# yumingj/Text2Human

Measured on NVIDIA H100. Metric: 512x256 images/sec VQ enc-quant-dec (vqvae_top), higher is better.
Workload: dtype f32 (fp16x3 split products, fp32 accumulate)

## Files before the change

### include/t2h.h

```cpp
#ifndef T2H_H_
#define T2H_H_

#include <stdint.h>

#ifdef __cplusplus
extern "C" {
#endif

#define T2H_VERSION 202

#define T2H_OK 0
#define T2H_EINVAL (-1)
#define T2H_ECUDA (-2)
#define T2H_EARCH (-3)

typedef void* t2h_stream_t;

int t2h_version(void);
const char* t2h_last_error(void);
int t2h_device_info(int* cc_major, int* cc_minor, int* num_sms);

#define T2H_MAX_TAPS 16

#define T2H_OUT_F32 0
// ... 9 lines not shown
#define T2H_ACT_LRELU 3

typedef struct t2h_tapgemm_params {
  const void* a;
  int32_t a_terms;
  int32_t a_term_imgs;
  int32_t a_imgs;
  int32_t a_bcast;
  int32_t n_img, H, W;
  int32_t tile_rows;
  int32_t a_H, a_W;
  int32_t C;
  int64_t a_sw, a_sh, a_sn;
  const void* b;
  int32_t b_terms;
  int32_t b_term_g;
  int32_t b_groups;
  int32_t b_groups2;
  int32_t b_batched;
  int32_t b_batched_h;
  int32_t n_out;
  int64_t b_sn, b_sg, b_sg2;
  int32_t ntaps;
  int32_t tap_dy[T2H_MAX_TAPS];
  int32_t tap_dx[T2H_MAX_TAPS];
  int32_t tap_img_off[T2H_MAX_TAPS];
  int32_t nterms;
  void* d;
  int32_t d_mode;
  int32_t d_terms;
  int64_t d_plane;
  int64_t d_sn, d_sh, d_sw, d_sc;
  const float* bias;
  int32_t bias_mode;
  int32_t act;
  float alpha;
  const float* residual;
  double* gn_stats;
  int32_t gn_cpg;
  int32_t a_mn;
  int32_t b_mn;
  int64_t bias_sn;
  int32_t k_split;
  int32_t use_tap_w;
  int32_t tap_w[T2H_MAX_TAPS];
  int32_t accumulate;
  int32_t k_partials;
  int64_t d_slab;
  double* nb_sums;
  const double* nb_stats;
  const float* nb_gamma;
  const float* nb_beta;
  float nb_eps;
  int32_t nb_act;
  int32_t nb_groups;
} t2h_tapgemm_params;

int t2h_tapgemm(const t2h_tapgemm_params* p, t2h_stream_t stream);
int t2h_debug_read(long long* out, int n);

int t2h_nchw_to_planes(const float* x, void* out, int n, int c, int h, int w,
                       int c_pad, int terms, t2h_stream_t stream);
int t2h_nhwc_to_nchw(const float* x, float* out, int n, int c, int h, int w,
                     t2h_stream_t stream);
int t2h_pack_u8(const float* x, uint8_t* out, int n, int c, int h, int w, float scale, float shift,
                t2h_stream_t stream);
int t2h_nchw_to_nhwc(const float* x, float* out, int n, int c, int h, int w,
                     t2h_stream_t stream);

#define T2H_CVT_PLAIN 0
#define T2H_CVT_UP2X 1
#define T2H_CVT_S2D 2
#define T2H_CVT_MAXPOOL2 3
#define T2H_CVT_BILINEAR2X 4
int t2h_f32_to_planes(const float* x, void* out, int n, int h, int w, int c,
                      int mode, int terms, t2h_stream_t stream);

int t2h_gn_stats(const float* x, double* stats, int n, int hw, int c, int groups,
                 t2h_stream_t stream);
int t2h_gn_apply(const float* x, const double* stats, const float* gamma,
                 const float* beta, void* out, int n, int hw, int c, int groups,
                 float eps, int swish, int terms, t2h_stream_t stream);

int t2h_add_inplace(float* x, const float* y, int64_t numel, t2h_stream_t stream);

int t2h_softmax_rows(const float* s, void* out, int64_t rows, int cols, float scale,
                     int terms, t2h_stream_t stream);

int t2h_attn_fwd(const void* qkv, int terms, int64_t plane, int64_t ld, int64_t rows, int q_col, int k_col,
                 int v_col, int batch, int tokens, int heads, int head_dim, float scale, void* out,
                 int64_t out_plane, int64_t ld_out, t2h_stream_t stream);

int t2h_vq_search(const float* z, const float* codebook, const int32_t* book_id,
                  int b, int hz, int wz, int cz, int ps, int n_books, int n_e,
                  int64_t cont_stride, int64_t* idx, int64_t* idx_cont,
                  int64_t* idx_list, float* zq_nhwc, float* zq_nchw, double* sqerr,
                  void* workspace, int64_t workspace_bytes, t2h_stream_t stream);
int64_t t2h_vq_workspace_bytes(int64_t rows, int n_books, int n_e);

int t2h_vq_gather(const float* codebook, const int64_t* idx, const int32_t* book_id,
                  int b, int hz, int wz, int cz, int ps, int n_books, int n_e,
                  float* zq_nhwc, float* zq_nchw, t2h_stream_t stream);

int t2h_onehot_to_planes(const float* ids, void* out, int b, int h, int w, int n_classes, int c_pad, int terms,
                         t2h_stream_t stream);

int t2h_texture_mask(const float* segm, const int32_t* attrs, const int32_t* cls_group, int n_cls, float* mask, int b,
                     int64_t per_img, t2h_stream_t stream);
int t2h_u8_to_planes(const uint8_t* x, void* out, float* nchw, int b, int h, int w, int c, int c_pad, float divisor,
                     float shift, int terms, t2h_stream_t stream);

int t2h_mask_to_ids(const float* mask, int32_t* ids, int b, int hs, int ws, int ht,
                    int wt, t2h_stream_t stream);

int t2h_argmax_heads(const float* logits, const int64_t* head, int64_t* out, int64_t rows, int n_heads, int ncls,
                     t2h_stream_t stream);

int t2h_embed_sum(const int64_t* idx, const int64_t* segm, const int64_t* tex,
                  const float* tok_emb, const float* pos_emb, const float* segm_emb,
                  const float* tex_emb, float* x, int b, int t, int c,
                  t2h_stream_t stream);
int t2h_layernorm(const float* x, const float* gamma, const float* beta, void* out,
                  int64_t rows, int c, float eps, int terms, t2h_stream_t stream);
int t2h_layernorm_scatter(const float* x, const float* gamma, const float* beta, void* out, int64_t rows, int c,
                          float eps, int terms, const int64_t* row_map, int64_t out_rows, t2h_stream_t stream);

int t2h_splitk_reduce_ln(const float* partials, int n_slabs, int64_t slab, const float* bias, const float* residual,
                         float* x_out, const float* gamma, const float* beta, float eps, void* ln_out, int terms,
                         const int64_t* row_map, int64_t ln_rows, int64_t rows, int c, t2h_stream_t stream);

int t2h_f32_to_planes_t(const float* x, void* out_t, void* out_n, int g, int r, int c, int terms, float scale,
                        t2h_stream_t stream);
int t2h_planes_transpose(const void* x, void* out, int g, int r, int c, int64_t ld, int64_t g_stride,
                         int64_t in_plane, int64_t out_ld, int64_t out_g_stride, int64_t out_plane, int terms,
                         t2h_stream_t stream);
int t2h_colsum(const float* x, float* out, int64_t rows, int c, t2h_stream_t stream);
int t2h_gelu_fwd(const float* a, void* out, int64_t n, int terms, t2h_stream_t stream);
int t2h_gelu_bwd(const float* a, const float* dg, float* da, void* da_planes ,
                 int64_t n, int terms, t2h_stream_t stream);
int t2h_layernorm_bwd(const float* dy, const float* x, const float* gamma, float* dx, float* dgamma,
                      float* dbeta, int64_t rows, int c, float eps, int accumulate, t2h_stream_t stream);
int t2h_layernorm_bwd_fused(const float* dy, const float* x, const float* gamma, float* dx, float* dgamma,
                            float* dbeta, int64_t rows, int c, float eps, int accumulate, void* dx_planes, int terms,
                            float* dx_colsum, t2h_stream_t stream);
int t2h_softmax_bwd(const void* p, const float* dp, float* ds, int64_t rows, int cols, float scale, int terms,
                    t2h_stream_t stream);
int t2h_softmax_bwd_planes(const void* p, const float* dp, void* ds_planes, int64_t rows, int cols, float scale,
                           int terms, float out_scale, t2h_stream_t stream);
int t2h_ce_heads(const float* logits, const int64_t* target, const int64_t* head, const float* w,
                 float* loss_rows, float* dlogits, int64_t rows, int nh, int ncls, t2h_stream_t stream);
int t2h_embed_bwd(const float* dx, const int64_t* idx, float* de, int64_t rows, int c, int t_mod,
                  t2h_stream_t stream);
int t2h_adam(float* p, const float* g, float* m, float* v, int64_t n, float lr, float beta1, float beta2,
             float eps, int step, float grad_scale, t2h_stream_t stream);

typedef struct t2h_conv_wgrad_params {
  const void* dy;
  int32_t dy_terms, dy_term_imgs, dy_imgs;
  int32_t n_img, H, W, cout;
  int64_t dy_sw, dy_sh, dy_sn;
  const void* x;
  int32_t x_terms, x_term_imgs, x_imgs;
  int32_t x_H, x_W, cin;
  int64_t x_sw, x_sh, x_sn;
  int32_t ntaps;
  int32_t tap_dy[T2H_MAX_TAPS], tap_dx[T2H_MAX_TAPS], tap_img_off[T2H_MAX_TAPS];
// ... 44 lines not shown
```

### text2human_b200/_lib.py

```python
import ctypes as C
import os

_HERE = os.path.dirname(os.path.abspath(__file__))
LIB_PATH = os.path.join(_HERE, "libt2h.so")

ABI_VERSION = 202
MAX_TAPS = 16
OUT_F32, OUT_PLANES = 0, 1
BIAS_NONE, BIAS_COL, BIAS_ROW = 0, 1, 2
ACT_NONE, ACT_GELU, ACT_RELU, ACT_LRELU = 0, 1, 2, 3
CVT_PLAIN, CVT_UP2X, CVT_S2D, CVT_MAXPOOL2, CVT_BILINEAR2X = 0, 1, 2, 3, 4


class TapGemmParams(C.Structure):
    _fields_ = [
        ("a", C.c_void_p), ("a_terms", C.c_int32), ("a_term_imgs", C.c_int32),
        ("a_imgs", C.c_int32), ("a_bcast", C.c_int32),
        ("n_img", C.c_int32), ("H", C.c_int32), ("W", C.c_int32), ("tile_rows", C.c_int32),
        ("a_H", C.c_int32), ("a_W", C.c_int32), ("C", C.c_int32),
        ("a_sw", C.c_int64), ("a_sh", C.c_int64), ("a_sn", C.c_int64),
        ("b", C.c_void_p), ("b_terms", C.c_int32), ("b_term_g", C.c_int32),
        ("b_groups", C.c_int32), ("b_groups2", C.c_int32), ("b_batched", C.c_int32),
        ("b_batched_h", C.c_int32), ("n_out", C.c_int32),
        ("b_sn", C.c_int64), ("b_sg", C.c_int64), ("b_sg2", C.c_int64),
        ("ntaps", C.c_int32),
        ("tap_dy", C.c_int32 * MAX_TAPS), ("tap_dx", C.c_int32 * MAX_TAPS),
        ("tap_img_off", C.c_int32 * MAX_TAPS),
        ("nterms", C.c_int32),
        ("d", C.c_void_p), ("d_mode", C.c_int32), ("d_terms", C.c_int32),
        ("d_plane", C.c_int64),
        ("d_sn", C.c_int64), ("d_sh", C.c_int64), ("d_sw", C.c_int64), ("d_sc", C.c_int64),
        ("bias", C.c_void_p), ("bias_mode", C.c_int32), ("act", C.c_int32),
        ("alpha", C.c_float),
        ("residual", C.c_void_p),
        ("gn_stats", C.c_void_p), ("gn_cpg", C.c_int32), ("a_mn", C.c_int32), ("b_mn", C.c_int32), ("bias_sn", C.c_int64), ("k_split", C.c_int32),
        ("use_tap_w", C.c_int32), ("tap_w", C.c_int32 * MAX_TAPS), ("accumulate", C.c_int32),
        ("k_partials", C.c_int32), ("d_slab", C.c_int64),
        ("nb_sums", C.c_void_p), ("nb_stats", C.c_void_p), ("nb_gamma", C.c_void_p), ("nb_beta", C.c_void_p),
        ("nb_eps", C.c_float), ("nb_act", C.c_int32), ("nb_groups", C.c_int32),
    ]


class ConvWgradParams(C.Structure):
    _fields_ = [
        ("dy", C.c_void_p), ("dy_terms", C.c_int32), ("dy_term_imgs", C.c_int32), ("dy_imgs", C.c_int32),
        ("n_img", C.c_int32), ("H", C.c_int32), ("W", C.c_int32), ("cout", C.c_int32),
        ("dy_sw", C.c_int64), ("dy_sh", C.c_int64), ("dy_sn", C.c_int64),
        ("x", C.c_void_p), ("x_terms", C.c_int32), ("x_term_imgs", C.c_int32), ("x_imgs", C.c_int32),
        ("x_H", C.c_int32), ("x_W", C.c_int32), ("cin", C.c_int32),
        ("x_sw", C.c_int64), ("x_sh", C.c_int64), ("x_sn", C.c_int64),
        ("ntaps", C.c_int32),
        ("tap_dy", C.c_int32 * MAX_TAPS), ("tap_dx", C.c_int32 * MAX_TAPS), ("tap_img_off", C.c_int32 * MAX_TAPS),
        ("dw", C.c_void_p), ("dw_tap_stride", C.c_int64), ("dw_ld", C.c_int64),
        ("alpha", C.c_float), ("nterms", C.c_int32), ("k_split", C.c_int32),
    ]


_I, _L, _P, _F = C.c_int, C.c_int64, C.c_void_p, C.c_float
SIGNATURES = {
    "t2h_version": (_I, []),
    "t2h_last_error": (C.c_char_p, []),
    "t2h_device_info": (_I, [C.POINTER(_I)] * 3),
    "t2h_tapgemm": (_I, [C.POINTER(TapGemmParams), _P]),
    "t2h_debug_read": (_I, [C.POINTER(C.c_longlong), _I]),
    "t2h_nchw_to_planes": (_I, [_P, _P, _I, _I, _I, _I, _I, _I, _P]),
    "t2h_nhwc_to_nchw": (_I, [_P, _P, _I, _I, _I, _I, _P]),
    "t2h_nchw_to_nhwc": (_I, [_P, _P, _I, _I, _I, _I, _P]),
    "t2h_f32_to_planes": (_I, [_P, _P, _I, _I, _I, _I, _I, _I, _P]),
    "t2h_gn_stats": (_I, [_P, _P, _I, _I, _I, _I, _P]),
    "t2h_gn_apply": (_I, [_P, _P, _P, _P, _P, _I, _I, _I, _I, _F, _I, _I, _P]),
    "t2h_add_inplace": (_I, [_P, _P, _L, _P]),
    "t2h_softmax_rows": (_I, [_P, _P, _L, _I, _F, _I, _P]),
    "t2h_attn_fwd": (_I, [_P, _I, _L, _L, _L, _I, _I, _I, _I, _I, _I, _I, _F, _P, _L, _L, _P]),
    "t2h_vq_search": (_I, [_P, _P, _P, _I, _I, _I, _I, _I, _I, _I, _L, _P, _P, _P, _P, _P, _P,
                           _P, _L, _P]),
    "t2h_vq_workspace_bytes": (_L, [_L, _I, _I]),
    "t2h_vq_gather": (_I, [_P, _P, _P, _I, _I, _I, _I, _I, _I, _I, _P, _P, _P]),
    "t2h_texture_mask": (_I, [_P, _P, _P, _I, _P, _I, _L, _P]),
    "t2h_u8_to_planes": (_I, [_P, _P, _P, _I, _I, _I, _I, _I, _F, _F, _I, _P]),
    "t2h_mask_to_ids": (_I, [_P, _P, _I, _I, _I, _I, _I, _P]),
    "t2h_onehot_to_planes": (_I, [_P, _P, _I, _I, _I, _I, _I, _I, _P]),
    "t2h_embed_sum": (_I, [_P, _P, _P, _P, _P, _P, _P, _P, _I, _I, _I, _P]),
    "t2h_layernorm": (_I, [_P, _P, _P, _P, _L, _I, _F, _I, _P]),
    "t2h_layernorm_scatter": (_I, [_P, _P, _P, _P, _L, _I, _F, _I, _P, _L, _P]),
    "t2h_splitk_reduce_ln": (_I, [_P, _I, _L, _P, _P, _P, _P, _P, _F, _P, _I, _P, _L, _L, _I, _P]),
    "t2h_pack_u8": (_I, [_P, _P, _I, _I, _I, _I, _F, _F, _P]),
    "t2h_argmax_heads": (_I, [_P, _P, _P, _L, _I, _I, _P]),
    "t2h_f32_to_planes_t": (_I, [_P, _P, _P, _I, _I, _I, _I, _F, _P]),
    "t2h_planes_transpose": (_I, [_P, _P, _I, _I, _I, _L, _L, _L, _L, _L, _L, _I, _P]),
    "t2h_colsum": (_I, [_P, _P, _L, _I, _P]),
    "t2h_gelu_fwd": (_I, [_P, _P, _L, _I, _P]),
    "t2h_gelu_bwd": (_I, [_P, _P, _P, _P, _L, _I, _P]),
    "t2h_layernorm_bwd_fused": (_I, [_P, _P, _P, _P, _P, _P, _L, _I, _F, _I, _P, _I, _P, _P]),
    "t2h_softmax_bwd_planes": (_I, [_P, _P, _P, _L, _I, _F, _I, _F, _P]),
    "t2h_layernorm_bwd": (_I, [_P, _P, _P, _P, _P, _P, _L, _I, _F, _I, _P]),
    "t2h_softmax_bwd": (_I, [_P, _P, _P, _L, _I, _F, _I, _P]),
    "t2h_ce_heads": (_I, [_P, _P, _P, _P, _P, _P, _L, _I, _I, _P]),
    "t2h_embed_bwd": (_I, [_P, _P, _P, _L, _I, _I, _P]),
    "t2h_adam": (_I, [_P, _P, _P, _P, _L, _F, _F, _F, _F, _I, _F, _P]),
    "t2h_conv_wgrad": (_I, [C.POINTER(ConvWgradParams), _P]),
    "t2h_norm_bwd": (_I, [_P, _P, _P, _P, _P, _P, _P, _P, _I, _P, _P, _P, _I, _I, _I, _I, _F, _I, _P, _I, _P]),
    "t2h_bn_update_running": (_I, [_P, _P, _P, _L, _F, _I, _P]),
    "t2h_lrelu_bwd": (_I, [_P, _P, _P, _P, _I, _L, _P]),
    "t2h_sumpool2": (_I, [_P, _P, _I, _I, _I, _I, _P]),
    "t2h_planes_s2d": (_I, [_P, _P, _I, _I, _I, _I, _I, _P]),
    "t2h_vq_bwd": (_I, [_P, _P, _P, _P, _P, _P, _P, _L, _I, _I, _I, _F, _F, _P]),
    "t2h_l1_loss": (_I, [_P, _P, _P, _P, _L, _F, _P]),
    "t2h_bce_logits": (_I, [_P, _P, _I, _I, _I, _I, _I, _F, _P, _P, _I, _P, _P]),
    "t2h_hinge_loss": (_I, [_P, _P, _P, _L, _F, _F, _P]),
    "t2h_diffaug_fwd": (_I, [_P, _P, _P, _P, _P, _I, _I, _I, _P]),
    "t2h_diffaug_bwd": (_I, [_P, _P, _P, _P, _P, _I, _I, _I, _P]),
    "t2h_adaptive_weight": (_I, [_P, _P, _L, _F, _F, _F, _P, _P]),
    "t2h_axpy_dev": (_I, [_P, _P, _P, _P, _L, _P]),
    "t2h_sample_step": (_I, [_P, _P, _P, _P, _P, _L, _I, _I, _F, _F, C.c_uint64, C.c_uint32, _L, _P]),
}

_lib = None


class T2HError(RuntimeError):
    pass


def load():
    global _lib
    if _lib is not None:
        return _lib
    if not os.path.exists(LIB_PATH):
        raise T2HError(
            f"{LIB_PATH} not found: build it with `python -c 'import __graft_entry__ as g; g.build()'` "
            "(or `make -C text2human_b200/csrc`). There is no CPU fallback.")
    lib = C.CDLL(LIB_PATH)
    for name, (res, args) in SIGNATURES.items():
        fn = getattr(lib, name)
        fn.restype = res
        fn.argtypes = args
    _lib = lib
    return lib


def check(rc):
    if rc != 0:
        raise T2HError(f"libt2h error {rc}: {load().t2h_last_error().decode()}")
```

### text2human_b200/ops.py

```python
import ctypes as C

import torch

from . import _lib
from ._lib import (ACT_GELU, ACT_LRELU, ACT_NONE, ACT_RELU, CVT_BILINEAR2X, CVT_MAXPOOL2, BIAS_COL, BIAS_NONE, BIAS_ROW, CVT_PLAIN, CVT_S2D, CVT_UP2X,
                   OUT_F32, OUT_PLANES, TapGemmParams)

_PRECISION = {"terms": 2, "mixed": False}


def set_precision(mode):
    _PRECISION["mixed"] = False
    if mode in ("fp32", "fp16x3", "exact"):
        _PRECISION["terms"] = 2
    elif mode in ("fp16", "fast", "tf32"):
        _PRECISION["terms"] = 1
    elif mode == "mixed":
        _PRECISION["terms"] = 2
        _PRECISION["mixed"] = True
    else:
        raise ValueError(f"unknown precision mode {mode!r}")


def layer_terms(mod):
# ... 353 lines not shown
    assert K == Kb and a.stride(3) == 1 and b.stride(3) == 1
    assert (Ga == G) or (a_bcast and Ga == 1)
    out = _alloc_out((G, M, N), planes_out, T, a.device)
    a_sn = a.stride(1)
    a_term_imgs = 1 if T == 1 else a.stride(0) // a_sn
    assert T == 1 or a.stride(0) % a_sn == 0
    _tapgemm(a=a, a_term_imgs=a_term_imgs, a_imgs=(T - 1) * a_term_imgs + Ga, a_bcast=1 if a_bcast else 0,
             n_img=G, H=1, W=M, a_H=1, a_W=M, Cc=K, a_sw=a.stride(2), a_sh=a_sn, a_sn=a_sn,
             b=b, b_term_g=1, b_groups=Tb, b_sg=b.stride(0), b_groups2=G, b_sg2=b.stride(1), b_batched=1,
             n_out=N, b_sn=b.stride(2),
             taps=_TAPS_1, d=out, d_mode=OUT_PLANES if planes_out else OUT_F32,
             d_strides=(M * N, 0, N, 1), d_plane=G * M * N,
             bias=bias_row if bias_col is None else bias_col,
             bias_mode=BIAS_ROW if bias_col is None else BIAS_COL,
             bias_sn=0 if bias_col is None else N, alpha=alpha, act=act)
    return out


def mha_scores(q, B, Tn, nh, alpha=1.0, k=None):
    if k is None:
        Cc = q.shape[2] // 2
        q, k = q[:, :, :Cc], q[:, :, Cc:]
    _need_cuda(q, k)
    T, M, Cc = q.shape
    hs = Cc // nh
    assert M == B * Tn and k.shape == q.shape and q.stride(2) == 1 and k.stride(2) == 1
    ldq, ldk = q.stride(1), k.stride(1)
    out = torch.empty((B, nh, Tn, Tn), dtype=torch.float32, device=q.device)
    plane = q.stride(0)
    assert plane % hs == 0 and (T == 1 or k.stride(0) == M * ldk)
    _tapgemm(a=q, a_term_imgs=plane // hs, a_imgs=(T - 1) * (plane // hs) + nh, a_bcast=0,
             n_img=nh, H=B, W=Tn, a_H=B, a_W=Tn, Cc=hs, a_sw=ldq, a_sh=Tn * ldq, a_sn=hs, tile_rows=1,
             b=k, b_term_g=B, b_groups=T * B, b_sg=Tn * ldk, b_batched_h=1,
             b_groups2=nh, b_sg2=hs, b_batched=1, n_out=Tn, b_sn=ldk,
             taps=_TAPS_1, d=out, d_mode=OUT_F32, d_strides=(Tn * Tn, nh * Tn * Tn, Tn, 1), alpha=alpha)
    return out


def mha_pv(p, vt, B, Tn, nh, out=None, planes_out=True, alpha=1.0, p_mn=False, v_tok=False):
    _need_cuda(p, vt)
    T = p.shape[0]
    assert p.is_contiguous()
    if v_tok:
        Cc = vt.shape[2]
        ldv = vt.stride(1)
        assert vt.shape[1] == B * Tn and vt.stride(2) == 1 and (T == 1 or vt.stride(0) == B * Tn * ldv)
        b_kw = dict(b_sg=Tn * ldv, b_sg2=Cc // nh, b_sn=ldv, b_mn=1)
    else:
        Cc = vt.shape[2]
        assert vt.is_contiguous()
        b_kw = dict(b_sg=Cc * Tn, b_sg2=(Cc // nh) * Tn, b_sn=Tn, b_mn=0)
    hs = Cc // nh
    if out is None:
        out = _alloc_out((B * Tn, Cc), planes_out, T, p.device)
    ld = out.stride(-2)
    _tapgemm(a=p, a_term_imgs=B * nh, a_imgs=T * B * nh, a_bcast=0,
             n_img=nh, H=B, W=Tn, a_H=B, a_W=Tn, Cc=Tn, a_sw=Tn, a_sh=nh * Tn * Tn, a_sn=Tn * Tn,
             tile_rows=1,
             b=vt, b_term_g=B, b_groups=T * B, b_batched_h=1,
             b_groups2=nh, b_batched=1, n_out=hs,
             taps=_TAPS_1, d=out, d_mode=OUT_PLANES if planes_out else OUT_F32, d_strides=(hs, Tn * ld, ld, 1),
             d_plane=out.stride(0) if planes_out else 0, alpha=alpha, a_mn=1 if p_mn else 0, **b_kw)
    return out


def split_planes(x, terms):
    x = x.detach().float()
    hi = x.half()
    if terms == 1:
        return hi.unsqueeze(0).contiguous()
    lo = (x - hi.float()).half()
    return torch.stack((hi, lo)).contiguous()


def pack_conv_weight(w, terms, c_pad=None):
    Cout, Cin, kh, kw = w.shape
    wt = w.detach().float().permute(2, 3, 0, 1).reshape(kh * kw, Cout, Cin)
    cp = c_pad if c_pad is not None else (Cin + 7) // 8 * 8
    if cp != Cin:
        wt = torch.nn.functional.pad(wt, (0, cp - Cin))
    return split_planes(wt, terms)


def conv_weight_for_dgrad(w):
    return w.detach().flip(2, 3).transpose(0, 1).contiguous()


def pack_linear_weight(w, terms):
    w2 = w.detach().float().reshape(w.shape[0], -1)
    return split_planes(w2.unsqueeze(0), terms)


def nchw_to_planes(x, c_pad=None, terms=None):
    _need_cuda(x)
    x = _f32c(x)
    N, Cc, H, W = x.shape
    terms = terms or get_terms()
    cp = c_pad if c_pad is not None else (Cc + 7) // 8 * 8
    out = torch.empty((terms, N, H, W, cp), dtype=torch.float16, device=x.device)
    _count(1)
    _lib.check(_lib.load().t2h_nchw_to_planes(_ptr(x), _ptr(out), N, Cc, H, W, cp, terms, _stream()))
    return out


def nhwc_to_nchw(x):
    _need_cuda(x)
    N, H, W, Cc = x.shape
    out = torch.empty((N, Cc, H, W), dtype=torch.float32, device=x.device)
    _count(1)
    _lib.check(_lib.load().t2h_nhwc_to_nchw(_ptr(x), _ptr(out), N, Cc, H, W, _stream()))
    return out


def nchw_to_nhwc(x):
    _need_cuda(x)
    x = _f32c(x)
    N, Cc, H, W = x.shape
    out = torch.empty((N, H, W, Cc), dtype=torch.float32, device=x.device)
    _count(1)
    _lib.check(_lib.load().t2h_nchw_to_nhwc(_ptr(x), _ptr(out), N, Cc, H, W, _stream()))
    return out


def f32_to_planes(x, mode=CVT_PLAIN, terms=None):
    _need_cuda(x)
    N, H, W, Cc = x.shape
    terms = terms or get_terms()
    if mode in (CVT_UP2X, CVT_BILINEAR2X):
        shape = (terms, N, 2 * H, 2 * W, Cc)
    elif mode == CVT_MAXPOOL2:
        shape = (terms, N, H // 2, W // 2, Cc)
    elif mode == CVT_S2D:
        shape = (terms, 4, N, H // 2, W // 2, Cc)
    else:
        shape = (terms, N, H, W, Cc)
    out = torch.empty(shape, dtype=torch.float16, device=x.device)
    _count(1)
    _lib.check(_lib.load().t2h_f32_to_planes(_ptr(x), _ptr(out), N, H, W, Cc, mode, terms, _stream()))
    return out


def group_norm(x, gamma, beta, *, swish, groups=32, eps=1e-6, terms=None, stats=None):
    _need_cuda(x)
    N, H, W, Cc = x.shape
    terms = terms or get_terms()
    lib = _lib.load()
    _count(1)
    if stats is None:
        stats = torch.zeros((N, groups, 2), dtype=torch.float64, device=x.device)
        _count(1)
        _lib.check(lib.t2h_gn_stats(_ptr(x), _ptr(stats), N, H * W, Cc, groups, _stream()))
    out = torch.empty((terms, N, H, W, Cc), dtype=torch.float16, device=x.device)
    _lib.check(lib.t2h_gn_apply(_ptr(x), _ptr(stats), _ptr(gamma), _ptr(beta), _ptr(out), N, H * W, Cc,
                                groups, eps, 1 if swish else 0, terms, _stream()))
    return out


def add_inplace(x, y):
    _need_cuda(x, y)
    assert x.shape == y.shape and x.is_contiguous() and y.is_contiguous()
    _count(1)
    _lib.check(_lib.load().t2h_add_inplace(_ptr(x), _ptr(y), x.numel(), _stream()))
    return x


def softmax_rows(s, scale=1.0, terms=None):
    _need_cuda(s)
    terms = terms or get_terms()
    cols = s.shape[-1]
    rows = s.numel() // cols
    out = torch.empty((terms,) + tuple(s.shape), dtype=torch.float16, device=s.device)
    _count(1)
    _lib.check(_lib.load().t2h_softmax_rows(_ptr(s), _ptr(out), rows, cols, scale, terms, _stream()))
    return out


FUSED_ATTN = {"on": _os_env.environ.get("T2H_FUSED_ATTN", "1") != "0"}


def set_fused_attn(on):
    old = FUSED_ATTN["on"]
    FUSED_ATTN["on"] = bool(on)
    return old


def can_fuse_attn(tokens, head_dim):
    return FUSED_ATTN["on"] and head_dim == 64 and tokens % 128 == 0 and 128 <= tokens <= 512


def attn_fused(qkv, B, Tn, nh, scale, out=None):
    _need_cuda(qkv)
    T, M, C3 = qkv.shape
    Cc = C3 // 3
    assert M == B * Tn and Cc == nh * 64 and qkv.stride(2) == 1 and qkv.dtype == torch.float16
    if out is None:
        out = torch.empty((T, M, Cc), dtype=torch.float16, device=qkv.device)
    assert out.shape == (T, M, Cc) and out.stride(2) == 1
    _count(1)
    _lib.check(_lib.load().t2h_attn_fwd(_ptr(qkv), T, qkv.stride(0), qkv.stride(1), M, 0, Cc, 2 * Cc, B, Tn, nh, 64,
                                        float(scale), _ptr(out), out.stride(0), out.stride(1), _stream()))
    return out


def layer_norm(x, gamma, beta, eps=1e-5, terms=None):
    _need_cuda(x)
    terms = terms or get_terms()
    rows, Cc = x.shape
    out = torch.empty((terms, rows, Cc), dtype=torch.float16, device=x.device)
    _count(1)
    _lib.check(_lib.load().t2h_layernorm(_ptr(x), _ptr(gamma), _ptr(beta), _ptr(out), rows, Cc, eps, terms,
                                         _stream()))
    return out


def layer_norm_scatter(x, gamma, beta, out, row_map, eps=1e-5):
    _need_cuda(x, out, row_map)
    rows, Cc = x.shape
    assert out.is_contiguous() and out.shape[2] == Cc and row_map.dtype == torch.int64 and row_map.numel() == rows
    _count(1)
    _lib.check(_lib.load().t2h_layernorm_scatter(_ptr(x), _ptr(gamma), _ptr(beta), _ptr(out), rows, Cc, eps,
                                                 out.shape[0], _ptr(row_map), out.shape[1], _stream()))
    return out


def embed_sum(idx, segm, tex, tok_emb, pos_emb, segm_emb, tex_emb):
    _need_cuda(idx, tok_emb)
    B, T = idx.shape
    Cc = tok_emb.shape[1]
    x = torch.empty((B * T, Cc), dtype=torch.float32, device=idx.device)
    _count(1)
    _lib.check(_lib.load().t2h_embed_sum(_ptr(idx.contiguous()), _ptr(segm.contiguous()),
                                         _ptr(tex.contiguous()), _ptr(tok_emb), _ptr(pos_emb),
                                         _ptr(segm_emb), _ptr(tex_emb), _ptr(x), B, T, Cc, _stream()))
    return x


def onehot_to_planes(segm, n_classes, terms=None):
# ... 499 lines not shown
```

### text2human_b200/vqgan_arch.py

```python
import numpy as np
import torch
import torch.nn as nn

from . import ops
from .ops import CVT_PLAIN, CVT_S2D, CVT_UP2X


def _cached(owner, key, params, build):
    cache = owner.__dict__.setdefault("_t2h_cache", {})
    sig = tuple((p.data_ptr(), p._version, str(p.device)) for p in params)
    hit = cache.get(key)
    if hit is not None and hit[0] == sig:
        return hit[1]
    with torch.no_grad():
        val = build()
    cache[key] = (sig, val)
    return val


def _conv_w(conv, c_pad=None):
    t = ops.layer_terms(conv)
    return _cached(conv, ("w3", t, c_pad), (conv.weight,),
                   lambda: ops.pack_conv_weight(conv.weight, t, c_pad))

# ... 92 lines not shown
        out_channels = in_channels if out_channels is None else out_channels
        self.out_channels = out_channels
        self.use_conv_shortcut = conv_shortcut

        self.norm1 = Normalize(in_channels)
        self.conv1 = torch.nn.Conv2d(in_channels, out_channels, kernel_size=3, stride=1, padding=1)
        if temb_channels > 0:
            self.temb_proj = torch.nn.Linear(temb_channels, out_channels)
        self.norm2 = Normalize(out_channels)
        self.dropout = torch.nn.Dropout(dropout)
        self.conv2 = torch.nn.Conv2d(out_channels, out_channels, kernel_size=3, stride=1, padding=1)
        if self.in_channels != self.out_channels:
            if self.use_conv_shortcut:
                self.conv_shortcut = torch.nn.Conv2d(in_channels, out_channels, kernel_size=3, stride=1,
                                                     padding=1)
            else:
                self.nin_shortcut = torch.nn.Conv2d(in_channels, out_channels, kernel_size=1, stride=1,
                                                    padding=0)

    def _fwd(self, act):
        assert self.dropout.p == 0.0 or not self.training, "dropout>0 in training is not implemented"
        x = act.x
        h = _Act(*_gn_conv3x3(act, self.norm1, self.conv1, want_stats=True))
        if self.in_channels != self.out_channels:
            xp = ops.f32_to_planes(x, CVT_PLAIN)
            if self.use_conv_shortcut:
                x = ops.conv3x3(xp, _conv_w(self.conv_shortcut), _f32(self.conv_shortcut.bias))
            else:
                x = conv1x1_nhwc(None, self.nin_shortcut, planes_in=xp)
        return _Act(*_gn_conv3x3(h, self.norm2, self.conv2, residual=x, want_stats=True))

    def forward_nhwc(self, x, temb=None):
        assert temb is None, "temb is always None on the Text2Human path (temb_ch=0)"
        return self._fwd(_Act(x)).x

    def forward(self, x, temb=None):
        return ops.nhwc_to_nchw(self.forward_nhwc(ops.nchw_to_nhwc(x), temb))


class AttnBlock(nn.Module):

    def __init__(self, in_channels):
        super().__init__()
        self.in_channels = in_channels
        self.norm = Normalize(in_channels)
        self.q = torch.nn.Conv2d(in_channels, in_channels, kernel_size=1, stride=1, padding=0)
        self.k = torch.nn.Conv2d(in_channels, in_channels, kernel_size=1, stride=1, padding=0)
        self.v = torch.nn.Conv2d(in_channels, in_channels, kernel_size=1, stride=1, padding=0)
        self.proj_out = torch.nn.Conv2d(in_channels, in_channels, kernel_size=1, stride=1, padding=0)

    def _qk_packed(self):
        t = ops.get_terms()
        w = _cached(self, ("wqk", t), (self.q.weight, self.k.weight),
                    lambda: ops.pack_linear_weight(torch.cat((self.q.weight, self.k.weight), 0), t))
        b = _cached(self, ("bqk",), (self.q.bias, self.k.bias),
                    lambda: torch.cat((self.q.bias, self.k.bias), 0).float().contiguous())
        return w, b

    def _fwd(self, act):
        x = act.x
        N, H, W, Cc = x.shape
        HW = H * W
        hn = _gn(act, self.norm, swish=False)
        T = hn.shape[0]
        wqk, bqk = self._qk_packed()
        qk = ops.linear(hn.reshape(T, N * HW, Cc), wqk, bqk, planes_out=True).view(T, N, HW, 2 * Cc)
        q, k = qk[..., :Cc], qk[..., Cc:]
        vt = ops.bmm_nt(_lin_w(self.v), hn.view(T, N, HW, Cc), planes_out=True,
                        bias_row=_f32(self.v.bias), a_bcast=True)
        s = ops.bmm_nt(q, k)
        p = ops.softmax_rows(s, scale=float(int(Cc) ** (-0.5)))
        o = ops.bmm_nt(p, vt, planes_out=True)
        return _Act(*ops.conv1x1(o.view(T, N, H, W, Cc), _lin_w(self.proj_out), _f32(self.proj_out.bias),
                                 residual=x, want_stats=True))

    def forward_nhwc(self, x):
        return self._fwd(_Act(x)).x

    def forward(self, x):
        return ops.nhwc_to_nchw(self.forward_nhwc(ops.nchw_to_nhwc(x)))


def _conv_in_nchw(conv, x):
    a = ops.nchw_to_planes(x)
    return _Act(*ops.conv3x3(a, _conv_w(conv, a.shape[-1]), _f32(conv.bias), want_stats=True))


def _conv_in_nhwc(conv, x):
    a = ops.f32_to_planes(x, CVT_PLAIN)
    return _Act(*ops.conv3x3(a, _conv_w(conv), _f32(conv.bias), want_stats=True))


def _conv_out(norm, conv, act, nchw):
    return _gn_conv3x3(act, norm, conv, nchw_out=nchw)


class Encoder(nn.Module):

    def __init__(self, ch, num_res_blocks, attn_resolutions, in_channels, resolution, z_channels,
                 ch_mult=(1, 2, 4, 8), dropout=0.0, resamp_with_conv=True, double_z=True):
        super().__init__()
        self.ch = ch
        self.temb_ch = 0
        self.num_resolutions = len(ch_mult)
        self.num_res_blocks = num_res_blocks
        self.resolution = resolution
        self.in_channels = in_channels

        self.conv_in = torch.nn.Conv2d(in_channels, self.ch, kernel_size=3, stride=1, padding=1)

        curr_res = resolution
        in_ch_mult = (1, ) + tuple(ch_mult)
        self.down = nn.ModuleList()
        for i_level in range(self.num_resolutions):
            block = nn.ModuleList()
            attn = nn.ModuleList()
            block_in = ch * in_ch_mult[i_level]
            block_out = ch * ch_mult[i_level]
            for _ in range(self.num_res_blocks):
                block.append(ResnetBlock(in_channels=block_in, out_channels=block_out,
                                         temb_channels=self.temb_ch, dropout=dropout))
                block_in = block_out
                if curr_res in attn_resolutions:
                    attn.append(AttnBlock(block_in))
            down = nn.Module()
            down.block = block
            down.attn = attn
            if i_level != self.num_resolutions - 1:
                down.downsample = Downsample(block_in, resamp_with_conv)
                curr_res = curr_res // 2
            self.down.append(down)

        self.mid = nn.Module()
        self.mid.block_1 = ResnetBlock(in_channels=block_in, out_channels=block_in,
                                       temb_channels=self.temb_ch, dropout=dropout)
        self.mid.attn_1 = AttnBlock(block_in)
        self.mid.block_2 = ResnetBlock(in_channels=block_in, out_channels=block_in,
                                       temb_channels=self.temb_ch, dropout=dropout)

        self.norm_out = Normalize(block_in)
        self.conv_out = torch.nn.Conv2d(block_in, 2 * z_channels if double_z else z_channels,
                                        kernel_size=3, stride=1, padding=1)

    def _body(self, h):
        for i_level in range(self.num_resolutions):
            lvl = self.down[i_level]
            for i_block in range(self.num_res_blocks):
                h = lvl.block[i_block]._fwd(h)
                if len(lvl.attn) > 0:
                    h = lvl.attn[i_block]._fwd(h)
            if i_level != self.num_resolutions - 1:
                h = lvl.downsample._fwd(h)
        h = self.mid.block_1._fwd(h)
        h = self.mid.attn_1._fwd(h)
        h = self.mid.block_2._fwd(h)
        return h

    @torch.no_grad()
    def forward_planes(self, a):
        h = _Act(*ops.conv3x3(a, _conv_w(self.conv_in, a.shape[-1]), _f32(self.conv_in.bias), want_stats=True))
        return _conv_out(self.norm_out, self.conv_out, self._body(h), nchw=False)

    @torch.no_grad()
    def forward_nhwc(self, x_nchw):
        h = self._body(_conv_in_nchw(self.conv_in, x_nchw))
        return _conv_out(self.norm_out, self.conv_out, h, nchw=False)

    def forward(self, x):
        from . import vqgan_autograd as VA
        if VA.recording(self, x):
            return VA.encoder_forward(self, x)
        with torch.no_grad():
            h = self._body(_conv_in_nchw(self.conv_in, x))
            return _conv_out(self.norm_out, self.conv_out, h, nchw=True)


# ... 334 lines not shown
```

Measured before the change: 201.5.

## Add fused GN-swish small-Cout conv and im2col path for first conv

For output convs with at most three channels, a new CUDA-core kernel fuses GroupNorm apply and swish with a direct fp32 3x3 convolution. This avoids materializing normalized fp16 planes and running a tensor-core GEMM that would waste most of its N dimension. For input convs with few channels, the NCHW input is turned into im2col fp16 planes so the conv runs as a single-tap GEMM with a dense K dimension instead of a padded 9-tap one. The small-Cout path computes in plain fp32 FMAs instead of split fp16 products, which shifts numerics slightly, and it adds an extra im2col buffer.

```diff
diff --git a/include/t2h.h b/include/t2h.h
--- a/include/t2h.h
+++ b/include/t2h.h
@@ -115,6 +115,13 @@
                  const float* beta, void* out, int n, int hw, int c, int groups,
                  float eps, int swish, int terms, t2h_stream_t stream);
 
+int t2h_gn_swish_conv3x3_small(const float* x, const double* stats, const float* gamma, const float* beta, float eps,
+                               const float* wpk, const float* bias, float* out, int n, int h, int w, int c, int cout,
+                               int groups, long long o_sn, long long o_sh, long long o_sw, long long o_sc,
+                               t2h_stream_t stream);
+int t2h_nchw_im2col_planes(const float* x, void* out, int n, int c, int h, int w, int k_pad, int terms,
+                           t2h_stream_t stream);
+
 int t2h_add_inplace(float* x, const float* y, int64_t numel, t2h_stream_t stream);
 
 int t2h_softmax_rows(const float* s, void* out, int64_t rows, int cols, float scale,
diff --git a/text2human_b200/_lib.py b/text2human_b200/_lib.py
--- a/text2human_b200/_lib.py
+++ b/text2human_b200/_lib.py
@@ -69,6 +69,8 @@
     "t2h_f32_to_planes": (_I, [_P, _P, _I, _I, _I, _I, _I, _I, _P]),
     "t2h_gn_stats": (_I, [_P, _P, _I, _I, _I, _I, _P]),
     "t2h_gn_apply": (_I, [_P, _P, _P, _P, _P, _I, _I, _I, _I, _F, _I, _I, _P]),
+    "t2h_gn_swish_conv3x3_small": (_I, [_P, _P, _P, _P, _F, _P, _P, _P, _I, _I, _I, _I, _I, _I, _L, _L, _L, _L, _P]),
+    "t2h_nchw_im2col_planes": (_I, [_P, _P, _I, _I, _I, _I, _I, _I, _P]),
     "t2h_add_inplace": (_I, [_P, _P, _L, _P]),
     "t2h_softmax_rows": (_I, [_P, _P, _L, _I, _F, _I, _P]),
     "t2h_attn_fwd": (_I, [_P, _I, _L, _L, _L, _I, _I, _I, _I, _I, _I, _I, _F, _P, _L, _L, _P]),
diff --git a/text2human_b200/csrc/conv_small.cu b/text2human_b200/csrc/conv_small.cu
--- /dev/null
+++ b/text2human_b200/csrc/conv_small.cu
@@ -0,0 +1,206 @@
+#include "t2h_internal.h"
+#include "t2h_ptx.cuh"
+
+namespace t2h {
+
+constexpr int kSW = 32, kSR = 8, kSWarps = 8, kSH = kSR * kSWarps, kSC = 8;
+constexpr int kSTileW = kSW + 2, kSTileH = kSH + 2, kSPix = kSTileW * kSTileH, kSPlane = kSPix;
+constexpr int kSThreads = kSWarps * 32;
+static_assert(kSPlane % 32 == 4 && kSC == 8, "activation plane stride: the two quads of a pixel 16 banks apart");
+
+template <int COUT>
+__global__ void __launch_bounds__(kSThreads, 3)
+gn_swish_conv3x3_small_kernel(const float* __restrict__ x, const double* __restrict__ stats,
+                              const float* __restrict__ gamma, const float* __restrict__ beta, float eps,
+                              const float* __restrict__ wpk, const float* __restrict__ bias, float* __restrict__ out,
+                              int H, int W, int C, int groups, long long o_sn, long long o_sh, long long o_sw,
+                              long long o_sc) {
+  extern __shared__ __align__(16) float sm[];
+  float* s_act = sm;
+  float* s_w = s_act + kSC * kSPlane;
+  float* s_scale = s_w + kSC * 36;
+  float* s_shift = s_scale + C;
+  const int n = blockIdx.z;
+  const int h0 = blockIdx.y * kSH, w0 = blockIdx.x * kSW;
+  const int tid = threadIdx.x, lane = tid & 31, warp = tid >> 5;
+
+  const int cpg = C / groups;
+  const double cnt = (double)H * W * cpg;
+  for (int c = tid; c < C; c += kSThreads) {
+    const int g = c / cpg;
+    const double s = stats[((long long)n * groups + g) * 2 + 0];
+    const double q = stats[((long long)n * groups + g) * 2 + 1];
+    const double mean = s / cnt;
+    double var = q / cnt - mean * mean;
+    if (var < 0) var = 0;
+    const float rstd = (float)(1.0 / sqrt(var + (double)eps));
+    const float ga = gamma[c] * rstd;
+    s_scale[c] = ga;
+    s_shift[c] = beta[c] - (float)mean * ga;
+  }
+
+  float acc[kSR][COUT];
+#pragma unroll
+  for (int o = 0; o < kSR; ++o)
+#pragma unroll
+    for (int co = 0; co < COUT; ++co) acc[o][co] = 0.f;
+
+  const float* xn = x + (long long)n * H * W * C;
+  for (int c0 = 0; c0 < C; c0 += kSC) {
+    __syncthreads();
+    for (int i = tid; i < kSC * 9; i += kSThreads)
+      reinterpret_cast<float4*>(s_w)[i] = __ldg(reinterpret_cast<const float4*>(wpk + (long long)c0 * 36) + i);
+#pragma unroll 4
+    for (int i = tid; i < kSPix * (kSC / 4); i += kSThreads) {
+      const int q = i & (kSC / 4 - 1), p = i / (kSC / 4);
+      const int r = p / kSTileW, col = p - r * kSTileW;
+      const int gh = h0 + r - 1, gw = w0 + col - 1;
+      float f[4] = {0.f, 0.f, 0.f, 0.f};
+      if (gh >= 0 && gh < H && gw >= 0 && gw < W) {
+        const float4 a = __ldg(reinterpret_cast<const float4*>(xn + ((long long)gh * W + gw) * C + c0) + q);
+        f[0] = a.x; f[1] = a.y; f[2] = a.z; f[3] = a.w;
+#pragma unroll
+        for (int e = 0; e < 4; ++e) {
+          const float y = f[e] * s_scale[c0 + 4 * q + e] + s_shift[c0 + 4 * q + e];
+          f[e] = y / (1.0f + __expf(-y));
+        }
+      }
+#pragma unroll
+      for (int e = 0; e < 4; ++e) s_act[(4 * q + e) * kSPlane + p] = f[e];
+    }
+    __syncthreads();
+#pragma unroll 1
+    for (int e = 0; e < kSC; ++e) {
+      float4 wv[9];
+#pragma unroll
+      for (int k = 0; k < 9; ++k) wv[k] = reinterpret_cast<const float4*>(s_w)[e * 9 + k];
+      const float* sp = s_act + e * kSPlane + warp * kSR * kSTileW + lane;
+#pragma unroll
+      for (int r = 0; r < kSR + 2; ++r) {
+        const float a0 = sp[r * kSTileW], a1 = sp[r * kSTileW + 1], a2 = sp[r * kSTileW + 2];
+#pragma unroll
+        for (int kh = 0; kh < 3; ++kh) {
+          const int o = r - kh;
+          if (o < 0 || o >= kSR) continue;
+#pragma unroll
+          for (int co = 0; co < COUT; ++co) {
+            const float* w0v = reinterpret_cast<const float*>(&wv[kh * 3 + 0]);
+            const float* w1v = reinterpret_cast<const float*>(&wv[kh * 3 + 1]);
+            const float* w2v = reinterpret_cast<const float*>(&wv[kh * 3 + 2]);
+            acc[o][co] = fmaf(a0, w0v[co], acc[o][co]);
+            acc[o][co] = fmaf(a1, w1v[co], acc[o][co]);
+            acc[o][co] = fmaf(a2, w2v[co], acc[o][co]);
+          }
+        }
+      }
+    }
+  }
+
+  const int gw = w0 + lane;
+  if (gw >= W) return;
+  float b[COUT];
+#pragma unroll
+  for (int co = 0; co < COUT; ++co) b[co] = bias[co];
+#pragma unroll
+  for (int o = 0; o < kSR; ++o) {
+    const int gh = h0 + warp * kSR + o;
+    if (gh < H) {
+      float* dst = out + n * o_sn + gh * o_sh + gw * o_sw;
+#pragma unroll
+      for (int co = 0; co < COUT; ++co) dst[co * o_sc] = acc[o][co] + b[co];
+    }
+  }
+}
+
+template <int COUT>
+static int launch_small(const float* x, const double* stats, const float* gamma, const float* beta, float eps,
+                        const float* wpk, const float* bias, float* out, int n, int h, int w, int c, int groups,
+                        long long o_sn, long long o_sh, long long o_sw, long long o_sc, cudaStream_t st) {
+  const size_t smem = (size_t)(kSC * kSPlane + kSC * 36 + 2 * c) * sizeof(float);
+  T2H_CUDA(cudaFuncSetAttribute(gn_swish_conv3x3_small_kernel<COUT>, cudaFuncAttributeMaxDynamicSharedMemorySize,
+                                (int)smem));
+  T2H_CUDA(cudaFuncSetAttribute(gn_swish_conv3x3_small_kernel<COUT>, cudaFuncAttributePreferredSharedMemoryCarveout,
+                                (int)cudaSharedmemCarveoutMaxShared));
+  dim3 grid(ceil_div(w, kSW), ceil_div(h, kSH), n);
+  gn_swish_conv3x3_small_kernel<COUT><<<grid, kSThreads, smem, st>>>(x, stats, gamma, beta, eps, wpk, bias, out, h, w,
+                                                                      c, groups, o_sn, o_sh, o_sw, o_sc);
+  T2H_LAUNCH_OK();
+  return T2H_OK;
+}
+
+struct alignas(16) Half8s {
+  __half v[8];
+};
+
+__global__ void nchw_im2col_planes_kernel(const float* __restrict__ x, __half* __restrict__ out, int N, int C, int H,
+                                          int W, int k_pad, int terms, long long plane) {
+  const int g8 = k_pad >> 3;
+  const long long total = (long long)N * H * W * g8;
+  const int K = 9 * C;
+  for (long long i = blockIdx.x * (long long)blockDim.x + threadIdx.x; i < total;
+       i += (long long)gridDim.x * blockDim.x) {
+    const long long pix = i / g8;
+    const int k0 = (int)(i - pix * g8) * 8;
+    const int w = (int)(pix % W);
+    const long long r = pix / W;
+    const int h = (int)(r % H);
+    const int n = (int)(r / H);
+    const float* xn = x + (long long)n * C * H * W;
+    Half8s hi, lo;
+    int tap = k0 / C, c = k0 - tap * C;
+#pragma unroll
+    for (int e = 0; e < 8; ++e) {
+      float v = 0.f;
+      if (k0 + e < K) {
+        const int ih = h + tap / 3 - 1, iw = w + tap % 3 - 1;
+        if (ih >= 0 && ih < H && iw >= 0 && iw < W) v = __ldg(xn + ((long long)c * H + ih) * W + iw);
+      }
+      split_f16(v, hi.v[e], lo.v[e]);
+      if (++c == C) { c = 0; ++tap; }
+    }
+    *reinterpret_cast<Half8s*>(out + i * 8) = hi;
+    if (terms == 2) *reinterpret_cast<Half8s*>(out + plane + i * 8) = lo;
+  }
+}
+
+}
+
+using namespace t2h;
+
+extern "C" {
+
+int t2h_gn_swish_conv3x3_small(const float* x, const double* stats, const float* gamma, const float* beta, float eps,
+                               const float* wpk, const float* bias, float* out, int n, int h, int w, int c, int cout,
+                               int groups, long long o_sn, long long o_sh, long long o_sw, long long o_sc,
+                               t2h_stream_t stream) {
+  T2H_CHECK_ARG(x && stats && gamma && beta && wpk && bias && out && n > 0 && h > 0 && w > 0,
+                "gn_swish_conv3x3_small: bad args");
+  T2H_CHECK_ARG(c % kSC == 0 && groups > 0 && c % groups == 0 && c <= 4096,
+                "gn_swish_conv3x3_small: C=%d groups=%d unsupported (C %% %d == 0 needed)", c, groups, kSC);
+  T2H_CHECK_ARG(cout >= 1 && cout <= 3, "gn_swish_conv3x3_small: Cout=%d must be 1..3", cout);
+  T2H_CHECK_ARG(reinterpret_cast<uintptr_t>(x) % 16 == 0 && reinterpret_cast<uintptr_t>(wpk) % 16 == 0,
+                "gn_swish_conv3x3_small: x and the packed weight must be 16-byte aligned");
+  cudaStream_t st = as_stream(stream);
+  switch (cout) {
+    case 1: return launch_small<1>(x, stats, gamma, beta, eps, wpk, bias, out, n, h, w, c, groups, o_sn, o_sh, o_sw, o_sc, st);
+    case 2: return launch_small<2>(x, stats, gamma, beta, eps, wpk, bias, out, n, h, w, c, groups, o_sn, o_sh, o_sw, o_sc, st);
+    default: return launch_small<3>(x, stats, gamma, beta, eps, wpk, bias, out, n, h, w, c, groups, o_sn, o_sh, o_sw, o_sc, st);
+  }
+}
+
+int t2h_nchw_im2col_planes(const float* x, void* out, int n, int c, int h, int w, int k_pad, int terms,
+                           t2h_stream_t stream) {
+  T2H_CHECK_ARG(x && out && n > 0 && c > 0 && h > 0 && w > 0, "nchw_im2col_planes: bad shape");
+  T2H_CHECK_ARG(k_pad >= 9 * c && k_pad % 8 == 0, "nchw_im2col_planes: k_pad=%d must be >= 9*C=%d and a multiple of 8",
+                k_pad, 9 * c);
+  T2H_CHECK_ARG(terms == 1 || terms == 2, "nchw_im2col_planes: terms=%d", terms);
+  T2H_CHECK_ARG(reinterpret_cast<uintptr_t>(out) % 16 == 0, "nchw_im2col_planes: output must be 16-byte aligned");
+  const long long pix = (long long)n * h * w;
+  const long long work = pix * (k_pad / 8);
+  nchw_im2col_planes_kernel<<<(unsigned)ceil_div64(work, 256), 256, 0, as_stream(stream)>>>(
+      x, reinterpret_cast<__half*>(out), n, c, h, w, k_pad, terms, pix * k_pad);
+  T2H_LAUNCH_OK();
+  return T2H_OK;
+}
+
+}
diff --git a/text2human_b200/ops.py b/text2human_b200/ops.py
--- a/text2human_b200/ops.py
+++ b/text2human_b200/ops.py
@@ -459,6 +459,21 @@
     return split_planes(wt, terms)
 
 
+def pack_conv_weight_im2col(w, terms, k_pad):
+    Cout, Cin, kh, kw = w.shape
+    wt = w.detach().float().permute(0, 2, 3, 1).reshape(1, Cout, kh * kw * Cin)
+    if k_pad != kh * kw * Cin:
+        wt = torch.nn.functional.pad(wt, (0, k_pad - kh * kw * Cin))
+    return split_planes(wt, terms)
+
+
+def pack_conv_weight_small(w):
+    Cout, Cin, kh, kw = w.shape
+    assert Cout <= 3 and kh == 3 and kw == 3, w.shape
+    wt = w.detach().float().permute(1, 2, 3, 0).reshape(Cin, 9, Cout)
+    return torch.nn.functional.pad(wt, (0, 4 - Cout)).contiguous()
+
+
 def conv_weight_for_dgrad(w):
     return w.detach().flip(2, 3).transpose(0, 1).contiguous()
 
@@ -477,6 +492,18 @@
     out = torch.empty((terms, N, H, W, cp), dtype=torch.float16, device=x.device)
     _count(1)
     _lib.check(_lib.load().t2h_nchw_to_planes(_ptr(x), _ptr(out), N, Cc, H, W, cp, terms, _stream()))
+    return out
+
+
+def nchw_im2col_planes(x, k_pad=None, terms=None):
+    _need_cuda(x)
+    x = _f32c(x)
+    N, Cc, H, W = x.shape
+    terms = terms or get_terms()
+    kp = k_pad if k_pad is not None else (9 * Cc + 31) // 32 * 32
+    out = torch.empty((terms, N, H, W, kp), dtype=torch.float16, device=x.device)
+    _count(1)
+    _lib.check(_lib.load().t2h_nchw_im2col_planes(_ptr(x), _ptr(out), N, Cc, H, W, kp, terms, _stream()))
     return out
 
 
@@ -530,6 +557,30 @@
     out = torch.empty((terms, N, H, W, Cc), dtype=torch.float16, device=x.device)
     _lib.check(lib.t2h_gn_apply(_ptr(x), _ptr(stats), _ptr(gamma), _ptr(beta), _ptr(out), N, H * W, Cc,
                                 groups, eps, 1 if swish else 0, terms, _stream()))
+    return out
+
+
+def gn_swish_conv3x3_small(x, gamma, beta, w_small, bias, *, groups=32, eps=1e-6, stats=None, nchw_out=True):
+    _need_cuda(x, w_small)
+    x = _f32c(x)
+    N, H, W, Cc = x.shape
+    Cout = bias.shape[0]
+    assert tuple(w_small.shape) == (Cc, 9, 4), (w_small.shape, x.shape)
+    lib = _lib.load()
+    if stats is None:
+        stats = torch.zeros((N, groups, 2), dtype=torch.float64, device=x.device)
+        _count(1)
+        _lib.check(lib.t2h_gn_stats(_ptr(x), _ptr(stats), N, H * W, Cc, groups, _stream()))
+    if nchw_out:
+        out = torch.empty((N, Cout, H, W), dtype=torch.float32, device=x.device)
+        strides = (Cout * H * W, W, 1, H * W)
+    else:
+        out = torch.empty((N, H, W, Cout), dtype=torch.float32, device=x.device)
+        strides = (H * W * Cout, W * Cout, Cout, 1)
+    _count(1)
+    _lib.check(lib.t2h_gn_swish_conv3x3_small(_ptr(x), _ptr(stats), _ptr(_f32c(gamma)), _ptr(_f32c(beta)), eps,
+                                              _ptr(w_small), _ptr(_f32c(bias)), _ptr(out), N, H, W, Cc, Cout, groups,
+                                              *strides, _stream()))
     return out
 
 
diff --git a/text2human_b200/vqgan_arch.py b/text2human_b200/vqgan_arch.py
--- a/text2human_b200/vqgan_arch.py
+++ b/text2human_b200/vqgan_arch.py
@@ -198,6 +198,12 @@
 
 
 def _conv_in_nchw(conv, x):
+    if 9 * conv.in_channels <= 64:
+        t = ops.layer_terms(conv)
+        a = ops.nchw_im2col_planes(x, terms=t)
+        kp = a.shape[-1]
+        w = _cached(conv, ("wi2c", t, kp), (conv.weight,), lambda: ops.pack_conv_weight_im2col(conv.weight, t, kp))
+        return _Act(*ops.conv3x3(a, w, _f32(conv.bias), want_stats=True, taps=ops._TAPS_1))
     a = ops.nchw_to_planes(x)
     return _Act(*ops.conv3x3(a, _conv_w(conv, a.shape[-1]), _f32(conv.bias), want_stats=True))
 
@@ -208,6 +214,11 @@
 
 
 def _conv_out(norm, conv, act, nchw):
+    if conv.out_channels <= 3:
+        w = _cached(conv, ("wsmall",), (conv.weight,), lambda: ops.pack_conv_weight_small(conv.weight))
+        stats = act.stats if norm.num_groups == ops.GN_GROUPS else None
+        return ops.gn_swish_conv3x3_small(act.x, _f32(norm.weight), _f32(norm.bias), w, _f32(conv.bias),
+                                          groups=norm.num_groups, eps=norm.eps, stats=stats, nchw_out=nchw)
     return _gn_conv3x3(act, norm, conv, nchw_out=nchw)
 
 
```

Measured after the change: 211.3 (median of 6 runs). 1.05x the previous value.
